# joyfang1106/MRLA

Measured on AMD Instinct MI355X. Metric: images/sec fwd+bwd resnet50_mrlal b=256, higher is better.
Workload: dtype bf16

## Files before the change

### include/mrla_hip.h

```cpp
#ifndef MRLA_HIP_H_
#define MRLA_HIP_H_

#include <stddef.h>
#include <stdint.h>

#ifdef __cplusplus
extern "C" {
#endif

#define MRLA_OK 0
#define MRLA_EINVAL (-1)
#define MRLA_EUNSUPPORTED (-2)
#define MRLA_EHIP (-3)

enum { MRLA_F32 = 0, MRLA_BF16 = 1, MRLA_F16 = 2 };
enum { MRLA_NCHW = 0, MRLA_NHWC = 1 };
enum { MRLA_ACT_NONE = 0, MRLA_ACT_GELU = 1 };
enum { MRLA_BN_NONE = 0, MRLA_BN_TRAIN = 1, MRLA_BN_EVAL = 2 };

#define MRLA_FWD_MOMENTS 8
#define MRLA_BWD_MOMENTS 3
#define MRLA_GEMM_MOMENTS 4

#define MRLA_ABI_VERSION 5
// ... 186 lines not shown
int mrla_conv1x1_rows(int m, int k, int n, int dtype);
int mrla_conv1x1_plan(int m, int k, int n, int dtype, int addend, int* out);
int mrla_conv1x1_fwd(const void* x, const void* w, void* y, float* mom_part, int m, int k, int n, int dtype, void* stream);

int mrla_conv1x1_add_supported(int m, int k, int n, int dtype);
int mrla_conv1x1_fwd_add(const void* x, const void* w, const void* addend, void* y, int m, int k, int n, int dtype,
                         void* stream);

int mrla_conv1x1_addend_supported(int m, int k, int n, int sh, int sw, int dtype);
int mrla_conv1x1_fwd_addend(const void* x, const void* w, const void* addend, void* y, int m, int k, int n, int b, int h,
                            int w_, int sh, int sw, int dtype, void* stream);

int mrla_conv1x1_fwd_affine_supported(int m, int k, int n, int dtype);
int mrla_conv1x1_fwd_affine(const void* x, const void* w, const float* sc, const float* sh, int relu, void* y, int m, int k,
                            int n, int dtype, void* stream);

int mrla_conv1x1_wgrad_rows(int m, int k, int n, int dtype);
int mrla_conv1x1_wgrad_plan(int m, int k, int n, int dtype, int* out);
int mrla_conv1x1_wgrad(const void* dy, const void* x, float* part, void* dw, int m, int k, int n, int dtype, int dw_dtype,
                       void* stream);

int mrla_conv1x1_wgrad_bn_supported(int m, int k, int n, int dtype);
int mrla_conv1x1_wgrad_bn(const void* g, const void* xb, const float* sc, const float* sh, const float* cb , int relu,
                          void* dy_out, const void* x, float* part, void* dw, int m, int k, int n, int dtype, int dw_dtype,
                          void* stream);

int mrla_conv1x1_wgrad_bn_dx_supported(int m, int k, int n, int dtype);
int mrla_conv1x1_wgrad_bn_dx(const void* g, const void* xb, const float* sc, const float* sh, const float* cb ,
                             int relu, const void* x, const void* wt , void* dx , float* part, void* dw,
                             int m, int k, int n, int dtype, int dw_dtype, void* stream);

int mrla_conv3x3_wgrad_rows(int b, int c, int n, int h, int w, int stride, int dtype);
int mrla_conv3x3_wgrad_plan(int b, int c, int n, int h, int w, int stride, int dtype, int* out);
int mrla_conv3x3_wgrad(const void* dy, const void* x, float* part, void* dw, int b, int c, int n, int h, int w,
                       int stride, int dtype, int dw_dtype, void* stream);

int mrla_conv3x3_fwd_rows(int b, int c, int n, int h, int w, int stride, int dtype);
int mrla_conv3x3_fwd_plan(int b, int c, int n, int h, int w, int stride, int dtype, int* out);
int mrla_conv3x3_fwd(const void* x, const void* wt, void* y, float* mom_part , int b, int c, int n, int h, int w,
                     int stride, int dtype, void* stream);

int mrla_conv3x3_dgrad_s2_plan(int b, int c, int n, int h, int w, int dtype, int* out);
int mrla_conv3x3_dgrad_s2(const void* dy, const void* wt, void* dx, int b, int c, int n, int h, int w, int dtype, void* stream);

int mrla_stem_conv_wgrad_rows(int b, int n, int h, int w, int dtype);
int mrla_stem_conv_wgrad_plan(int b, int n, int h, int w, int dtype, int* out);
int mrla_stem_conv_wgrad(const void* dy, const void* x, float* part, void* dw, int b, int n, int h, int w, int dtype,
                         int dw_dtype, void* stream);

int mrla_conv1x1_f32_rows(int m, int k, int n);
int mrla_conv1x1_f32_plan(int m, int k, int n, int* out);
int mrla_conv1x1_f32_fwd(const float* x, const float* w, int w_trans, float* y, float* mom_part , int m, int k, int n,
                         void* stream);
int mrla_conv1x1_f32_wgrad_rows(int m, int k, int n);
int mrla_conv1x1_f32_wgrad(const float* dy, const float* x, float* part, float* dw, int m, int k, int n, void* stream);

int mrla_weight_bank_refresh(const void* table, int entries, int max_tiles, void* stream);
int mrla_weight_bank_refresh_dt(const void* table, int entries, int max_tiles, int dtype, void* stream);

int mrla_reduce_rows(const float* in, float* out, int rows, int n, void* stream);
int mrla_reduce_rows2(const float* in1, float* out1, int rows1, int n1, const float* in2, float* out2, int rows2, int n2,
                      void* stream);



int mrla_light_tail_fwd(const void* x, const float* pre_sc, const float* pre_sh, const void* o_prev, const float* wq,
// ... 58 lines not shown
```

### mrla_amd/__init__.py

```python


def __getattr__(name):
    if name in ("graphed_step", "GraphedStep", "replay_matches_eager", "capture_step", "GraphReplayMismatch"):
        from . import graphs
        return getattr(graphs, name)
    if name == "fp32_gemms":
        from . import functional
        return functional.fp32_gemms
    if name == "conv3x3_wgrad":
        from . import functional
        return functional.conv3x3_wgrad
    if name == "conv3x3_fwd":
        from . import functional
        return functional.conv3x3_fwd
    if name == "conv3x3_dgrad":
        from . import functional
        return functional.conv3x3_dgrad
    if name == "stem_wgrad":
        from . import functional
        return functional.stem_wgrad
    if name == "reproducible_gradients":
        from . import functional
        return functional.reproducible_gradients
    raise AttributeError(f"module 'mrla_amd' has no attribute {name!r}")
```

### mrla_amd/_lib.py

```python
import ctypes
import os

_HERE = os.path.dirname(os.path.abspath(__file__))
LIB_PATH = os.environ.get("MRLA_HIP_LIB") or os.path.join(_HERE, "libmrla_hip.so")

ABI_VERSION = 5
OK, EINVAL, EUNSUPPORTED, EHIP = 0, -1, -2, -3
F32, BF16, F16 = 0, 1, 2
NCHW, NHWC = 0, 1
ACT_NONE, ACT_GELU = 0, 1
BN_NONE, BN_TRAIN, BN_EVAL = 0, 1, 2
FWD_MOMENTS, BWD_MOMENTS, TOKEN_PARTIALS, GEMM_MOMENTS = 8, 3, 15, 4

_ERR = {EINVAL: "invalid argument", EUNSUPPORTED: "unsupported shape/layout for the HIP kernels",
        EHIP: "HIP runtime error at kernel launch"}

_P, _I, _F = ctypes.c_void_p, ctypes.c_int, ctypes.c_float

SIGNATURES = {
    "mrla_abi_version": [],
    "mrla_light_wgrad_rows": [_I] * 6,
    "mrla_light_stats_fwd": [_P, _P, _P, _P, _I, _I, _I, _I, _I, _I, _I, _P],
    "mrla_light_gate_fwd": [_P, _P, _P, _I, _P, _I, _I, _I, _I, _P],
    "mrla_light_bn_fwd": [_P, _P, _P, _P, _P, _P, _P, _I, _F, _F, _P, _P, _P, _P, _I, _I, _I, _I, _P],
# ... 51 lines not shown
    "mrla_bn_relu_pool_fwd": [_P, _P, _P, _P, _I, _I, _I, _I, _I, _I, _P],
    "mrla_bn_relu_pool_dmoments": [_P, _P, _P, _P, _P, _P, _I, _I, _I, _I, _I, _I, _P],
    "mrla_bn_relu_pool_bwd": [_P, _P, _P, _P, _P, _P, _I, _I, _I, _I, _I, _I, _P],
    "mrla_bn_gate_supported": [_I] * 6,
    "mrla_bn_gate_pool": [_P] * 6 + [_I] * 5 + [_P],
    "mrla_eca_gate_fwd": [_P, _P, _I, _P, _I, _I, _P],
    "mrla_eca_gate_bwd": [_P, _P, _P, _P, _I, _P, _P, _P, _I, _I, _I, _P],
    "mrla_bn_gate_sums_bwd": [_P] * 9 + [_I] * 5 + [_P],
    "mrla_bn_gate_fwd": [_P, _P, _P, _P, _P] + [_I] * 6 + [_P],
    "mrla_bn_gate_bwd": [_P, _P, _P, _P, _P, _P] + [_I] * 6 + [_P],
    "mrla_conv1x1_rows": [_I] * 4,
    "mrla_conv1x1_plan": [_I, _I, _I, _I, _I, _P],
    "mrla_conv1x1_wgrad_plan": [_I, _I, _I, _I, _P],
    "mrla_conv1x1_fwd": [_P, _P, _P, _P, _I, _I, _I, _I, _P],
    "mrla_conv1x1_add_supported": [_I] * 4,
    "mrla_conv1x1_fwd_add": [_P, _P, _P, _P, _I, _I, _I, _I, _P],
    "mrla_conv1x1_addend_supported": [_I] * 6,
    "mrla_conv1x1_fwd_addend": [_P, _P, _P, _P] + [_I] * 9 + [_P],
    "mrla_conv1x1_fwd_affine_supported": [_I] * 4,
    "mrla_conv1x1_fwd_affine": [_P, _P, _P, _P, _I, _P, _I, _I, _I, _I, _P],
    "mrla_conv1x1_wgrad_rows": [_I] * 4,
    "mrla_conv1x1_wgrad": [_P, _P, _P, _P, _I, _I, _I, _I, _I, _P],
    "mrla_conv1x1_f32_rows": [_I] * 3,
    "mrla_conv1x1_f32_plan": [_I, _I, _I, _P],
    "mrla_conv1x1_f32_fwd": [_P, _P, _I, _P, _P, _I, _I, _I, _P],
    "mrla_conv1x1_f32_wgrad_rows": [_I] * 3,
    "mrla_conv1x1_f32_wgrad": [_P, _P, _P, _P, _I, _I, _I, _P],
    "mrla_conv1x1_wgrad_bn_supported": [_I] * 4,
    "mrla_conv1x1_wgrad_bn": [_P, _P, _P, _P, _P, _I, _P, _P, _P, _P, _I, _I, _I, _I, _I, _P],
    "mrla_conv1x1_wgrad_bn_dx_supported": [_I] * 4,
    "mrla_conv1x1_wgrad_bn_dx": [_P, _P, _P, _P, _P, _I, _P, _P, _P, _P, _P, _I, _I, _I, _I, _I, _P],
    "mrla_conv3x3_wgrad_rows": [_I] * 7,
    "mrla_conv3x3_wgrad_plan": [_I] * 7 + [_P],
    "mrla_conv3x3_wgrad": [_P, _P, _P, _P] + [_I] * 8 + [_P],
    "mrla_conv3x3_fwd_rows": [_I] * 7,
    "mrla_conv3x3_fwd_plan": [_I] * 7 + [_P],
    "mrla_conv3x3_fwd": [_P, _P, _P, _P] + [_I] * 7 + [_P],
    "mrla_conv3x3_dgrad_s2_plan": [_I] * 6 + [_P],
    "mrla_conv3x3_dgrad_s2": [_P, _P, _P] + [_I] * 6 + [_P],
    "mrla_stem_conv_wgrad_rows": [_I] * 5,
    "mrla_stem_conv_wgrad_plan": [_I] * 5 + [_P],
    "mrla_stem_conv_wgrad": [_P, _P, _P, _P] + [_I] * 6 + [_P],
    "mrla_weight_bank_refresh": [_P, _I, _I, _P],
    "mrla_weight_bank_refresh_dt": [_P, _I, _I, _I, _P],
    "mrla_reduce_rows": [_P, _P, _I, _I, _P],
    "mrla_reduce_rows2": [_P, _P, _I, _I, _P, _P, _I, _I, _P],
    "mrla_light_tail_fwd": [_P] * 6 + [_I] + [_P] * 6 + [_I, _F, _F] + [_P] * 6 + [_I] * 10 + [_P],
    "mrla_light_tail_bwd": [_P] * 5 + [_I] + [_P] * 7 + [_I] + [_P] * 5 + [_I] + [_P] * 8 + [_I] * 10 + [_P],
    "mrla_bn_fwd": [_P, _P, _I, _P, _P, _I, _P, _P, _P, _P, _I, _F, _F, _P, _I, _P] + [_I] * 6 + [_P],
    "mrla_bn_bwd": [_P] * 5 + [_I] * 4 + [_P, _P] + [_I] * 6 + [_P],
    "mrla_stem_fwd": [_P, _P, _P, _I, _P, _P, _P, _P, _I, _F, _F, _P, _P] + [_I] * 6 + [_P],
    "mrla_stem_bwd": [_P] * 5 + [_I, _I, _P, _P] + [_I] * 6 + [_P],
    "mrla_base_layer_fwd": [_P] * 6 + [_I] + [_P] * 5 + [_I, _F, _F] + [_P] * 9 + [_I] + [_P, _P] + [_I] * 9 + [_P],
    "mrla_base_layer_bwd": ([_P] * 5 + [_I] + [_P] * 6 + [_I] + [_P] * 6 + [_I] + [_P, _P] + [_I] + [_P] * 5 + [_I] + [_P] * 5
                            + [_I] * 12 + [_P]),
    "mrla_token_light_fwd": [_P] * 8 + [_I] + [_P, _P] + [_F] + [_P] * 4 + [_I] * 6 + [_P],
    "mrla_token_light_bwd": [_P] * 10 + [_I] + [_P] * 6 + [_I] + [_P] * 6 + [_I] * 6 + [_P],
}


class MrlaHipError(RuntimeError):
    pass


_lib = None

# ... 77 lines not shown
```

### mrla_amd/csrc/capi.hip

```cpp
#include <algorithm>
#include <atomic>
#include <mutex>

#include "mrla_device.h"
#include "mrla_kernels.h"

namespace mrla {

hipError_t lds_opt_in(const void* kernel, size_t bytes) {
  if (bytes <= 48 * 1024) return hipSuccess;
  constexpr unsigned kSlots = 1024;
  static std::atomic<uintptr_t> keys[kSlots];
  static std::atomic<int> granted[kSlots];
  static std::mutex raise_mutex;
  int dev = 0;
  if (hipGetDevice(&dev) != hipSuccess) return hipErrorInvalidDevice;
  const uintptr_t key = reinterpret_cast<uintptr_t>(kernel) ^ ((uintptr_t)(dev + 1) << 52);
  unsigned i = (unsigned)((key >> 4) * 0x9E3779B1u) % kSlots;
  int slot = -1;
  for (unsigned probe = 0; probe < kSlots; ++probe, i = (i + 1) % kSlots) {
    uintptr_t k = keys[i].load(std::memory_order_acquire);
    if (k == 0 && keys[i].compare_exchange_strong(k, key, std::memory_order_acq_rel)) k = key;
    if (k == key) { slot = (int)i; break; }
  }
// ... 712 lines not shown
  if ((dw_dtype == MRLA_F16 && dtype != MRLA_F16) || (dw_dtype == MRLA_BF16 && dtype == MRLA_F16)) return MRLA_EINVAL;
  if (dtype != MRLA_BF16 && dtype != MRLA_F16) return MRLA_EUNSUPPORTED;
  return launch_conv1x1_wgrad(dy, x, part, dw, dw_dtype == MRLA_F32, m, k, n, dtype, (hipStream_t)stream);
}

static int conv3x3_args(int b, int c, int n, int h, int w, int stride, int dtype) {
  if (b <= 0 || c <= 0 || n <= 0 || h <= 0 || w <= 0 || stride <= 0 || bad_dtype(dtype)) return MRLA_EINVAL;
  if (dtype != MRLA_BF16 && dtype != MRLA_F16) return MRLA_EUNSUPPORTED;
  return MRLA_OK;
}

static int stem_conv_wgrad_args(int b, int n, int h, int w, int dtype) { return conv3x3_args(b, 3, n, h, w, 2, dtype); }

static int wgrad_launch_args(const void* dy, const void* x, const void* part, const void* dw, int dtype, int dw_dtype, int rc) {
  if (!dy || !x || !part || !dw) return MRLA_EINVAL;
  if (((uintptr_t)dy | (uintptr_t)x | (uintptr_t)part | (uintptr_t)dw) & 15) return MRLA_EINVAL;
  if (dw_dtype != MRLA_BF16 && dw_dtype != MRLA_F16 && dw_dtype != MRLA_F32) return MRLA_EINVAL;
  if (rc == MRLA_EINVAL) return rc;
  if (dw_dtype != MRLA_F32 && dw_dtype != dtype) return MRLA_EINVAL;
  return rc;
}

int mrla_conv3x3_wgrad_rows(int b, int c, int n, int h, int w, int stride, int dtype) {
  const int rc = conv3x3_args(b, c, n, h, w, stride, dtype);
  return rc != MRLA_OK ? rc : conv3x3_wgrad_rows(b, c, n, h, w, stride);
}

int mrla_conv3x3_wgrad_plan(int b, int c, int n, int h, int w, int stride, int dtype, int* out) {
  if (!out) return MRLA_EINVAL;
  const int rc = conv3x3_args(b, c, n, h, w, stride, dtype);
  return rc != MRLA_OK ? rc : conv3x3_wgrad_plan(b, c, n, h, w, stride, out);
}

int mrla_conv3x3_wgrad(const void* dy, const void* x, float* part, void* dw, int b, int c, int n, int h, int w, int stride,
                       int dtype, int dw_dtype, void* stream) {
  const int rc = wgrad_launch_args(dy, x, part, dw, dtype, dw_dtype, conv3x3_args(b, c, n, h, w, stride, dtype));
  if (rc != MRLA_OK) return rc;
  return launch_conv3x3_wgrad(dy, x, part, dw, dw_dtype == MRLA_F32, b, c, n, h, w, stride, dtype, (hipStream_t)stream);
}

int mrla_conv3x3_fwd_rows(int b, int c, int n, int h, int w, int stride, int dtype) {
  const int rc = conv3x3_args(b, c, n, h, w, stride, dtype);
  return rc != MRLA_OK ? rc : conv3x3_fwd_rows(b, c, n, h, w, stride);
}

int mrla_conv3x3_fwd_plan(int b, int c, int n, int h, int w, int stride, int dtype, int* out) {
  if (!out) return MRLA_EINVAL;
  const int rc = conv3x3_args(b, c, n, h, w, stride, dtype);
  return rc != MRLA_OK ? rc : conv3x3_fwd_plan(b, c, n, h, w, stride, out);
}

int mrla_conv3x3_fwd(const void* x, const void* wt, void* y, float* mom_part, int b, int c, int n, int h, int w, int stride,
                     int dtype, void* stream) {
  if (!x || !wt || !y) return MRLA_EINVAL;
  if (((uintptr_t)x | (uintptr_t)wt | (uintptr_t)y | (uintptr_t)mom_part) & 15) return MRLA_EINVAL;
  const int rc = conv3x3_args(b, c, n, h, w, stride, dtype);
  if (rc != MRLA_OK) return rc;
  return launch_conv3x3_fwd(x, wt, y, mom_part, b, c, n, h, w, stride, dtype, (hipStream_t)stream);
}

int mrla_conv3x3_dgrad_s2_plan(int b, int c, int n, int h, int w, int dtype, int* out) {
  if (!out) return MRLA_EINVAL;
  const int rc = conv3x3_args(b, c, n, h, w, 2, dtype);
  return rc != MRLA_OK ? rc : conv3x3_dgrad_s2_plan(b, c, n, h, w, out);
}

// ... 180 lines not shown
```

### mrla_amd/csrc/conv3x3_wgrad.hip

```cpp
#include <algorithm>
#include <type_traits>

#include "conv_spatial.h"

namespace mrla {
namespace {

typedef c1_f32x16 c3_f32x16;

constexpr int kC3Tile = 64;
constexpr int kC3Waves = 4;
constexpr int kC3Stages = 1;
constexpr int kC3Target = 2 * 256;
constexpr int kC3MaxKP1 = 128;
constexpr int kC3MaxKP2 = 96;
constexpr int kC3MaxPY = 60;
static_assert(kTileRowB == kC3Tile * 2, "a tile row is one pixel, 64 channels");

struct C3Plan : Raster3x3 {
  int rows_per_split = 0, splits = 0, tiles = 0;
};

struct C3Args {
  int b, h, w, ho, wo, c, n;
  int py, ws, nseg, rmax, kp_cap;
  int rows_per_split, splits, tiles_c;
  float inv_py, inv_px;
};

__device__ __forceinline__ int c3_off(int row, int chunk) { return tile_off<1, 2>(row, chunk); }

template <typename T>
__device__ __forceinline__ typename Elem16<T>::x8 c3_frag(const unsigned char* tile, int r, int r2, int chunk, int sub) {
  return tr16_frag<T>(tile + c3_off(r, chunk) + sub, tile + c3_off(r2, chunk) + sub);
}

template <typename T, int S>
__device__ __forceinline__ void conv3x3_wgrad_body(const T* __restrict__ dY, const T* __restrict__ X, float* __restrict__ part,
                                                   const C3Args& a) {
#if defined(__HIP_DEVICE_COMPILE__)
  extern __shared__ __align__(16) unsigned char smem_raw[];
  unsigned char* const ty_tile = smem_raw;
  unsigned char* const tx_tile = smem_raw + a.kp_cap * kTileRowB;
  const int tid = threadIdx.x, lane = tid & (kWave - 1), wave = tid / kWave;
  const int tiles = (a.n / kC3Tile) * a.tiles_c;
  const int split = blockIdx.x / tiles, tile = blockIdx.x - split * tiles;
  const int tn = tile / a.tiles_c, tc = tile - tn * a.tiles_c;
  const int n0 = tn * kC3Tile, c0 = tc * kC3Tile;
  const int rows = a.b * a.ho;
  const int r_begin = split * a.rows_per_split, r_end = min(rows, r_begin + a.rows_per_split);
  const int PY = a.py, PX = S * a.py;

  const int wn = wave >> 1, wc = wave & 1;
  const int g = lane >> 4, q = (lane >> 2) & 3, pp = lane & 3;
  const int krel = 8 * (g >> 1) + q;
  const int colA = wn * 32 + 16 * (g & 1) + 4 * pp, colB = wc * 32 + 16 * (g & 1) + 4 * pp;
  const int chA = colA >> 3, subA = ((colA >> 2) & 1) * 8, chB = colB >> 3, subB = ((colB >> 2) & 1) * 8;

  c3_f32x16 acc[9];
#pragma unroll
  for (int t = 0; t < 9; ++t)
#pragma unroll
    for (int e = 0; e < 16; ++e) acc[t][e] = 0.f;

  const int prow = tid >> 3, pch = tid & 7;
  const u32x4 zero4 = {0u, 0u, 0u, 0u};

  for (int r = r_begin; r < r_end;) {
    const RowStep st = row_step(r, r_end, a.ho, a.rmax);
    const int img = st.img, yo0 = st.yo0, R = st.R;
    for (int seg = 0; seg < a.nseg; ++seg) {
      const int xo0 = seg * a.ws, ws = min(a.ws, a.wo - xo0);
      const int KP = (R * PY + 15) & ~15;
      const int XT = S * KP + S * (S - 1) * PY * (R - 1) + 2 * PX + 3;
      const int ty_need = S * (R - 1) + 3, cx_need = S * (ws - 1) + 3;
      const int yi0 = yo0 * S - 1, xi0 = xo0 * S - 1;
      __syncthreads();
      for (int p0 = 0; p0 < KP; p0 += 128) {
        u32x4 v[4];
#pragma unroll
        for (int u = 0; u < 4; ++u) {
          const int p = p0 + 32 * u + prow;
          const int ry = (int)(((float)p + 0.5f) * a.inv_py), j = p - ry * PY;
          v[u] = zero4;
          if (p < KP && ry < R && j < ws)
            v[u] = *reinterpret_cast<const u32x4*>(dY + ((size_t)((img * a.ho + yo0 + ry) * a.wo + xo0 + j) * a.n + n0 + pch * 8));
        }
#pragma unroll
        for (int u = 0; u < 4; ++u) {
          const int p = p0 + 32 * u + prow;
          if (p < KP) *reinterpret_cast<u32x4*>(ty_tile + c3_off(p, pch)) = v[u];
        }
      }
      for (int t0 = 0; t0 < XT; t0 += 128) {
        u32x4 v[4];
#pragma unroll
        for (int u = 0; u < 4; ++u) {
          const int t = t0 + 32 * u + prow;
          const int ty = (int)(((float)t + 0.5f) * a.inv_px), cx = t - ty * PX;
          const int yi = yi0 + ty, xi = xi0 + cx;
          v[u] = zero4;
          if (t < XT && ty < ty_need && cx < cx_need && yi >= 0 && yi < a.h && xi >= 0 && xi < a.w)
            v[u] = *reinterpret_cast<const u32x4*>(X + ((size_t)((img * a.h + yi) * a.w + xi) * a.c + c0 + pch * 8));
        }
#pragma unroll
        for (int u = 0; u < 4; ++u) {
          const int t = t0 + 32 * u + prow;
          if (t < XT) *reinterpret_cast<u32x4*>(tx_tile + c3_off(t, pch)) = v[u];
        }
      }
      __syncthreads();
      for (int k0 = 0; k0 < KP; k0 += 16) {
        const int k = k0 + krel;
        const typename Elem16<T>::x8 fa = c3_frag<T>(ty_tile, k, k + 4, chA, subA);
        int xr = S * k, xr2 = S * (k + 4);
        if (S > 1) {
          xr += S * (S - 1) * PY * min((int)(((float)k + 0.5f) * a.inv_py), R - 1);
          xr2 += S * (S - 1) * PY * min((int)(((float)k + 4.5f) * a.inv_py), R - 1);
        }
#pragma unroll
        for (int kh = 0; kh < 3; ++kh)
#pragma unroll
          for (int kw = 0; kw < 3; ++kw) {
            const typename Elem16<T>::x8 fb = c3_frag<T>(tx_tile, xr + kh * PX + kw, xr2 + kh * PX + kw, chB, subB);
            Elem16<T>::mfma(acc[kh * 3 + kw], fa, fb);
          }
      }
    }
    r += R;
  }

  float* po = part + (((size_t)split * a.n + n0 + wn * 32) * 9) * a.c + c0 + wc * 32 + (lane & 31);
  const int hh = lane >> 5;
#pragma unroll
  for (int t = 0; t < 9; ++t)
#pragma unroll
    for (int e = 0; e < 16; ++e) po[((size_t)(8 * (e >> 2) + 4 * hh + (e & 3)) * 9 + t) * a.c] = acc[t][e];
#endif
}

template <typename T, int S>
__global__ __launch_bounds__(kC3Waves* kWave, 2) void conv3x3_wgrad_kernel(const T* __restrict__ dY, const T* __restrict__ X,
                                                                           float* __restrict__ part, C3Args a) {
  conv3x3_wgrad_body<T, S>(dY, X, part, a);
}

C3Plan c3_plan(int b, int c, int n, int h, int w, int s) {
  C3Plan p;
  static_cast<Raster3x3&>(p) = raster3x3(b, c, n, h, w, s, kC3MaxKP1, kC3MaxKP2, kC3MaxPY, 16);
  if (!p.ok) return p;
  p.tiles = (n / kC3Tile) * (c / kC3Tile);
  const RowSplit sp = split_rows((long long)b * p.ho, p.tiles, kC3Target);
  p.rows_per_split = sp.per;
  p.splits = sp.count;
  return p;
}

template <typename T, int S>
int c3_launch(const C3Plan& p, const C3Args& a, const void* dy, const void* x, float* part, hipStream_t st) {
  const size_t lds = (size_t)(p.kp_cap + p.xt_cap) * kTileRowB;
  if (lds > 80 * 1024) return MRLA_EUNSUPPORTED;
  if (lds_opt_in(reinterpret_cast<const void*>(conv3x3_wgrad_kernel<T, S>), lds) != hipSuccess) return MRLA_EHIP;
  hipLaunchKernelGGL((conv3x3_wgrad_kernel<T, S>), dim3(p.tiles * p.splits), dim3(kC3Waves * kWave), lds, st, (const T*)dy,
                     (const T*)x, part, a);
  return MRLA_OK;
}

}

int conv3x3_wgrad_rows(int b, int c, int n, int h, int w, int s) {
  const C3Plan p = c3_plan(b, c, n, h, w, s);
  return p.ok ? p.splits : MRLA_EUNSUPPORTED;
}

int conv3x3_wgrad_plan(int b, int c, int n, int h, int w, int s, int* out) {
  const C3Plan p = c3_plan(b, c, n, h, w, s);
  if (!p.ok) return MRLA_EUNSUPPORTED;
  out[0] = kC3Tile; out[1] = kC3Tile; out[2] = p.rows_per_split; out[3] = kC3Stages; out[4] = p.splits; out[5] = p.tiles;
  return MRLA_OK;
}

int launch_conv3x3_wgrad(const void* dy, const void* x, float* part, void* dw, int dw_f32, int b, int c, int n, int h, int w,
                         int s, int dtype, hipStream_t st) {
  const C3Plan p = c3_plan(b, c, n, h, w, s);
  if (!p.ok || (dtype != MRLA_BF16 && dtype != MRLA_F16)) return MRLA_EUNSUPPORTED;
  C3Args a;
  a.b = b; a.h = h; a.w = w; a.ho = p.ho; a.wo = p.wo; a.c = c; a.n = n;
  a.py = p.py; a.ws = p.ws; a.nseg = p.nseg; a.rmax = p.rmax; a.kp_cap = p.kp_cap;
  a.rows_per_split = p.rows_per_split; a.splits = p.splits; a.tiles_c = c / kC3Tile;
  a.inv_py = 1.0f / (float)p.py; a.inv_px = 1.0f / (float)(s * p.py);
  int rc;
  if (dtype == MRLA_F16)
    rc = s == 1 ? c3_launch<f16_t, 1>(p, a, dy, x, part, st) : c3_launch<f16_t, 2>(p, a, dy, x, part, st);
  else
    rc = s == 1 ? c3_launch<bf16_t, 1>(p, a, dy, x, part, st) : c3_launch<bf16_t, 2>(p, a, dy, x, part, st);
  if (rc != MRLA_OK) return rc;
  return launch_split_sum(part, dw, dw_f32, dtype, p.splits, n * 9 * c, st);
}

}
```

### mrla_amd/csrc/mrla_kernels.h

```cpp
#pragma once
#include <hip/hip_runtime.h>
#include <stddef.h>
#include <stdint.h>

#include "../../include/mrla_hip.h"

namespace mrla {

constexpr int kMaxTasksPerWave = 4;

struct SlabGeo {
  int B, C, H, W, HW;
  int CP;
  int slabs;
  int WS;
  int PW;
  int NG;
  int NB;
  int RB;
  int BG;
  int astride;
};

inline size_t dtype_size(int dtype) { return dtype == MRLA_F32 ? 4 : 2; }
// ... 146 lines not shown
int launch_bn_relu_pool_bwd(const void* dp, const void* x, const float* sc, const float* sh, const float* cb, void* dx,
                            int B, int C, int H, int W, int dtype, hipStream_t st);
int conv1x1_wide_rows(int M, int K, int N);
int conv1x1_wide_plan(int M, int K, int N, int add, int* out);
int launch_conv1x1_wide(const void* x, const void* w, const void* addend, void* y, float* part, int M, int K, int N,
                        int dtype, hipStream_t st);
int launch_conv1x1_wide_sparse(const void* x, const void* w, const void* addend, void* y, int M, int K, int N, int b, int h,
                               int wd, int sh, int sw, int dtype, hipStream_t st);
int launch_conv1x1_wide_affine(const void* x, const void* w, const float* sc, const float* sh, int relu, void* y, int M, int K,
                               int N, int dtype, hipStream_t st);
int conv1x1_kstream_supported(int M, int K, int N);
int conv1x1_kstream_stages(int M, int K, int N);
int conv1x1_kstream_rows(int M, int K, int N);
int launch_conv1x1_kstream(const void* x, const void* w, void* y, float* part, int M, int K, int N, int dtype, hipStream_t st);
int launch_conv1x1_kstream_addend(const void* x, const void* w, const void* addend, void* y, int M, int K, int N, int b, int h,
                                  int wd, int sh, int sw, int dtype, hipStream_t st);
int launch_conv1x1_kstream_affine(const void* x, const void* w, const float* sc, const float* sh, int relu, void* y, int M,
                                  int K, int N, int dtype, hipStream_t st);
int conv1x1_wgrad_rows(int M, int K, int N);
int conv1x1_wgrad_plan(int M, int K, int N, int* out);
int launch_conv1x1_wgrad(const void* dy, const void* x, float* part, void* dw, int dw_f32, int M, int K, int N, int dtype,
                         hipStream_t st);
int conv1x1_wgrad_bn_supported(int M, int K, int N);
int launch_conv1x1_wgrad_bn(const void* g, const void* xb, const float* sc, const float* sh, const float* cb, int relu,
                            void* dy_out, const void* x, float* part, void* dw, int dw_f32, int M, int K, int N, int dtype,
                            hipStream_t st);
int conv1x1_wgrad_bn_dx_supported(int M, int K, int N);
int launch_conv1x1_wgrad_bn_dx(const void* g, const void* xb, const float* sc, const float* sh, const float* cb, int relu,
                               const void* x, const void* wt, void* dx, float* part, void* dw, int dw_f32, int M, int K, int N,
                               int dtype, hipStream_t st);
int launch_conv1x1_wgrad_reduce_f32(const float* part, float* dw, int splits, int NK, hipStream_t st);
int conv3x3_wgrad_rows(int b, int c, int n, int h, int w, int s);
int conv3x3_wgrad_plan(int b, int c, int n, int h, int w, int s, int* out);
int launch_conv3x3_wgrad(const void* dy, const void* x, float* part, void* dw, int dw_f32, int b, int c, int n, int h, int w,
                         int s, int dtype, hipStream_t st);
int conv3x3_fwd_rows(int b, int c, int n, int h, int w, int s);
int conv3x3_fwd_plan(int b, int c, int n, int h, int w, int s, int* out);
int launch_conv3x3_fwd(const void* x, const void* wt, void* y, float* mom, int b, int c, int n, int h, int w, int s, int dtype,
                       hipStream_t st);
int conv3x3_dgrad_s2_plan(int b, int c, int n, int h, int w, int* out);
int launch_conv3x3_dgrad_s2(const void* dy, const void* wt, void* dx, int b, int c, int n, int h, int w, int dtype,
                            hipStream_t st);
int stem_conv_wgrad_rows(int b, int n, int h, int w);
int stem_conv_wgrad_plan(int b, int n, int h, int w, int* out);
int launch_stem_conv_wgrad(const void* dy, const void* x, float* part, void* dw, int dw_f32, int b, int n, int h, int w,
                           int dtype, hipStream_t st);
int conv1x1_f32_rows(int M, int K, int N);
int conv1x1_f32_plan(int M, int K, int N, int* out);
int launch_conv1x1_f32_fwd(const float* x, const float* w, int w_trans, float* y, float* part, int M, int K, int N,
                           hipStream_t st);
int conv1x1_f32_wgrad_rows(int M, int K, int N);
int launch_conv1x1_f32_wgrad(const float* dy, const float* x, float* part, float* dw, int M, int K, int N, hipStream_t st);
int launch_weight_bank_refresh(const long long* table, int entries, int max_tiles, int dtype, hipStream_t st);
int launch_light_stats_fwd_wide(const void* x, const void* o, const float* wv, float* mom, void* xout, const float* psc,
                                const float* psh, void* vout, int B, int C, int H, int W, int dtype, int act,
                                hipStream_t st, bool fused_no_x = false, int mom_ranges = 1);
int launch_light_apply_fwd_wide(const void* x, const void* o, const float* wv, const float* gate, const float* sc,
                                const float* sh, const float* lam, const float* dp, void* out, int B, int C, int H,
                                int W, int d, int res, int dtype, int act, hipStream_t st);
int launch_light_apply_fwd_pre_wide(const void* pre, const void* o, const float* psc, const float* psh, const float* wv,
                                    const float* gate, const float* sc, const float* sh, const float* lam,
                                    const float* dp, void* out, int B, int C, int H, int W, int d, int res, int dtype,
                                    hipStream_t st);
int launch_light_apply_bwd_wide(const void* dout, const void* x, const void* o, const float* wv, const float* gate,
                                const float* cb, const float* lam, const float* dp, const float* dyx, void* dx,
                                void* dprev, float* dwv_part, const void* pre, const float* pre_center, float* pre_tmom,
// ... 50 lines not shown
```

### mrla_amd/functional.py

```python
import contextlib
import ctypes
import threading
import weakref
from math import log

import torch

from . import _lib as L

_DT = {torch.float32: L.F32, torch.bfloat16: L.BF16, torch.float16: L.F16}


def k_size_for(c):
    t = int(abs((log(c, 2) + 1) / 2.0))
    return t if t % 2 else t + 1


class KernelTimer:

    def __init__(self, names=None):
        self.names = None if names is None else set(names)
        self.records = []

    def summary(self):
# ... 15 lines not shown
LEAN = False


SHORTCUT_ADDEND = True


WGRAD_BN = True


CONV1X1_F32 = False


def _switch(flag, name):
    @contextlib.contextmanager
    def manager(enabled=True):
        g = globals()
        prev, g[flag] = g[flag], bool(enabled)
        try:
            yield
        finally:
            g[flag] = prev
    manager.__name__ = manager.__qualname__ = name
    manager.__doc__ = f"{flag} = `enabled` inside the block; the previous value comes back on exit, also when the block raises."
    return manager


fp32_gemms = _switch("CONV1X1_F32", "fp32_gemms")


CONV3X3_WGRAD = False


conv3x3_wgrad = _switch("CONV3X3_WGRAD", "conv3x3_wgrad")


CONV3X3_FWD = False


conv3x3_fwd = _switch("CONV3X3_FWD", "conv3x3_fwd")


CONV3X3_DGRAD = False


conv3x3_dgrad = _switch("CONV3X3_DGRAD", "conv3x3_dgrad")


STEM_WGRAD = False


stem_wgrad = _switch("STEM_WGRAD", "stem_wgrad")


@contextlib.contextmanager
def reproducible_gradients(enabled=True):
    with conv3x3_wgrad(enabled), stem_wgrad(enabled):
        yield


WGRAD_BN_DX = True


CHANNEL_GATE = True


EVAL_FOLD = True
# ... 1692 lines not shown
        return None
    n, (kh, kw, c) = dy.shape[1], taps
    part = torch.empty((rows, n, kh * kw * c), dtype=torch.float32, device=x.device)
    gw = torch.empty((n, c, kh, kw), dtype=ctx.wdtype, device=x.device, memory_format=_CL)
    _call(entry, (dy.numel() + x.numel()) * x.element_size(), _ptr(dy), _ptr(x), _ptr(part), _ptr(gw), *shape, dt,
          _DT[ctx.wdtype], _stream())
    return gw


def _stock_conv_backward(ctx, dy, x, w16, stride, padding, gx, gw):
    need_x, need_w = ctx.needs_input_grad[0] and gx is None, ctx.needs_input_grad[1] and gw is None
    if need_x or need_w:
        gx2, gw2, _ = torch.ops.aten.convolution_backward(dy, x, w16, None, stride, padding, (1, 1), False, (0, 0), 1,
                                                          [need_x, need_w, False])
        gx = gx2 if need_x else gx
        gw = gw2.to(ctx.wdtype) if need_w else gw
    return gx, gw


def _weight_strides(ctx, gw):
    if gw is not None and gw.stride() != ctx.wstride:
        gw = torch.empty_strided(ctx.wshape, ctx.wstride, dtype=gw.dtype, device=gw.device).copy_(gw)
    return gw


def conv3x3_applies(conv, x):
    dt = _spatial_conv_applies(conv, x, (3, 3), ((1, 1), (2, 2)), (1, 1), True)
    if dt is None:
        return False
    b, c, h, w = x.shape
    return L.load().mrla_conv3x3_wgrad_rows(b, c, conv.out_channels, h, w, conv.stride[0], _DT[dt]) > 0


def _own_dgrad_s2(dy, x, w16):
    b, c, h, wd = x.shape
    gx = torch.empty_like(x)
    _call("mrla_conv3x3_dgrad_s2", (dy.numel() + gx.numel()) * x.element_size(), _ptr(dy), _ptr(w16), _ptr(gx),
          b, c, w16.shape[0], h, wd, _DT[x.dtype], _stream())
    return gx


class _Conv3x3Fn(torch.autograd.Function):

    @staticmethod
    @_on_device
    def forward(ctx, x, w, stride, own_wgrad, own_dgrad):
        ctx.stride, ctx.own_wgrad, ctx.own_dgrad = (stride, stride), own_wgrad, own_dgrad
        ctx.wshape, ctx.wstride, ctx.wdtype = w.shape, w.stride(), w.dtype
        w16 = w if w.dtype == x.dtype else w.to(x.dtype)
        if own_dgrad:
            w16 = w16.contiguous(memory_format=_CL)
            if w16.data_ptr() % 16:
                w16 = w16.clone(memory_format=_CL)
        ctx.save_for_backward(x, w16)
        return torch.ops.aten.convolution(x, w16, None, ctx.stride, (1, 1), (1, 1), False, (0, 0), 1)

    @staticmethod
    @_on_device
    def backward(ctx, dy):
        x, w16 = ctx.saved_tensors
        dy = dy.contiguous(memory_format=_CL)
        b, c, h, wd = x.shape
        own = dy.dtype == x.dtype and dy.data_ptr() % 16 == 0
        gx = gw = None
        if ctx.needs_input_grad[1] and own and ctx.own_wgrad:
            gw = _own_wgrad(ctx, "mrla_conv3x3_wgrad", "mrla_conv3x3_wgrad_rows", dy, x,
# ... 44 lines not shown
              _ptr(part) if moments else None, b, c, n, h, wd, stride, dt, _stream())
        ctx.save_for_backward(x, w16)
        ctx.mark_non_differentiable(part)
        return y, part

    @staticmethod
    @_on_device
    def backward(ctx, dy, _dpart=None):
        if dy is None:
            return None, None, None, None, None, None
        x, w16 = ctx.saved_tensors
        need_x, need_w = ctx.needs_input_grad[0], ctx.needs_input_grad[1]
        dy = dy.contiguous(memory_format=_CL)
        b, c, h, wd = x.shape
        n, dt = w16.shape[0], _DT[x.dtype]
        own = dy.dtype == x.dtype and dy.data_ptr() % 16 == 0
        gx = gw = None
        if need_w and own and ctx.own_wgrad:
            gw = _own_wgrad(ctx, "mrla_conv3x3_wgrad", "mrla_conv3x3_wgrad_rows", dy, x, (b, c, n, h, wd, ctx.stride[0]), (3, 3, c))
        if need_x and own and ctx.stride[0] == 1:
            wflip = w16.flip(2, 3).transpose(0, 1).contiguous(memory_format=_CL)
            gx = torch.empty_like(x)
            _call("mrla_conv3x3_fwd", (dy.numel() + gx.numel()) * x.element_size(), _ptr(dy), _ptr(wflip), _ptr(gx), None,
                  b, n, c, h, wd, 1, dt, _stream())
        if need_x and own and ctx.own_dgrad:
            gx = _own_dgrad_s2(dy, x, w16)
        gx, gw = _stock_conv_backward(ctx, dy, x, w16, ctx.stride, (1, 1), gx, gw)
        return gx, _weight_strides(ctx, gw), None, None, None, None


def _conv3x3_own(x, conv, moments):
    dt = _conv_compute_dtype(x)
    return _Conv3x3FwdFn.apply(x if x.dtype == dt else x.to(dt), conv.weight, conv.stride[0], moments,
                               CONV3X3_WGRAD and conv3x3_applies(conv, x), CONV3X3_DGRAD and conv3x3_dgrad_applies(conv, x))


def conv3x3(x, conv):
    if CONV3X3_FWD and conv3x3_fwd_applies(conv, x):
        return _conv3x3_own(x, conv, False)[0]
    own_wgrad = CONV3X3_WGRAD and conv3x3_applies(conv, x)
    own_dgrad = CONV3X3_DGRAD and conv3x3_dgrad_applies(conv, x)
    if not (own_wgrad or own_dgrad):
        return conv(x)
    dt = _conv_compute_dtype(x)
    return _Conv3x3Fn.apply(x if x.dtype == dt else x.to(dt), conv.weight, conv.stride[0], own_wgrad, own_dgrad)


def conv3x3_bn_act(x, conv, bn, relu, defer=False):
    if CONV3X3_FWD and conv3x3_fwd_applies(conv, x):
        moments = type(bn) is torch.nn.BatchNorm2d and bn.affine and bn.track_running_stats and bn.training
        y, part = _conv3x3_own(x, conv, moments)
        return bn_act(y, bn, relu, defer, pre_moments=part if moments else None)
    return bn_act(conv3x3(x, conv), bn, relu, defer)


def stem_conv_applies(conv, x):
    dt = _spatial_conv_applies(conv, x, (7, 7), ((2, 2),), (3, 3), True)
    if dt is None or conv.in_channels != 3:
        return False
    b, _, h, w = x.shape
    return L.load().mrla_stem_conv_wgrad_rows(b, conv.out_channels, h, w, _DT[dt]) > 0


class _StemConvFn(torch.autograd.Function):

    @staticmethod
    @_on_device
    def forward(ctx, x, w):
        ctx.wshape, ctx.wstride, ctx.wdtype = w.shape, w.stride(), w.dtype
        w16 = w if w.dtype == x.dtype else w.to(x.dtype)
        ctx.save_for_backward(x, w16)
        return torch.ops.aten.convolution(x, w16, None, (2, 2), (3, 3), (1, 1), False, (0, 0), 1)

# ... 104 lines not shown
```

Before: 9181.

## Prefetch next conv3x3 wgrad step and auto-enable kernel for stride-1 shapes

Restructures the conv3x3 weight-gradient kernel so the dY and X tiles for the next row/segment step are loaded into registers while the current step's MFMAs run. For stride 1 the X raster comes entirely from that register prefetch. The stride-1 inner loop is rewritten to load the B fragment for the next tap ahead of its MFMA. A heuristic (steps ≥ 4, pixels ≥ 384, stride 1) exposed through a new C API now turns the custom wgrad on by default for stride-1 convs instead of the stock PyTorch backward. The trade-off is more register pressure and a dispatch decision cached per shape.

```diff
diff --git a/include/mrla_hip.h b/include/mrla_hip.h
--- a/include/mrla_hip.h
+++ b/include/mrla_hip.h
@@ -242,6 +242,7 @@
 
 int mrla_conv3x3_wgrad_rows(int b, int c, int n, int h, int w, int stride, int dtype);
 int mrla_conv3x3_wgrad_plan(int b, int c, int n, int h, int w, int stride, int dtype, int* out);
+int mrla_conv3x3_wgrad_preferred(int b, int c, int n, int h, int w, int stride, int dtype);
 int mrla_conv3x3_wgrad(const void* dy, const void* x, float* part, void* dw, int b, int c, int n, int h, int w,
                        int stride, int dtype, int dw_dtype, void* stream);
 
diff --git a/mrla_amd/__init__.py b/mrla_amd/__init__.py
--- a/mrla_amd/__init__.py
+++ b/mrla_amd/__init__.py
@@ -10,6 +10,9 @@
     if name == "conv3x3_wgrad":
         from . import functional
         return functional.conv3x3_wgrad
+    if name == "conv3x3_wgrad_auto":
+        from . import functional
+        return functional.conv3x3_wgrad_auto
     if name == "conv3x3_fwd":
         from . import functional
         return functional.conv3x3_fwd
diff --git a/mrla_amd/_lib.py b/mrla_amd/_lib.py
--- a/mrla_amd/_lib.py
+++ b/mrla_amd/_lib.py
@@ -107,6 +107,7 @@
     "mrla_conv1x1_wgrad_bn_dx": [_P, _P, _P, _P, _P, _I, _P, _P, _P, _P, _P, _I, _I, _I, _I, _I, _P],
     "mrla_conv3x3_wgrad_rows": [_I] * 7,
     "mrla_conv3x3_wgrad_plan": [_I] * 7 + [_P],
+    "mrla_conv3x3_wgrad_preferred": [_I] * 7,
     "mrla_conv3x3_wgrad": [_P, _P, _P, _P] + [_I] * 8 + [_P],
     "mrla_conv3x3_fwd_rows": [_I] * 7,
     "mrla_conv3x3_fwd_plan": [_I] * 7 + [_P],
diff --git a/mrla_amd/csrc/capi.hip b/mrla_amd/csrc/capi.hip
--- a/mrla_amd/csrc/capi.hip
+++ b/mrla_amd/csrc/capi.hip
@@ -768,6 +768,11 @@
   return rc != MRLA_OK ? rc : conv3x3_wgrad_plan(b, c, n, h, w, stride, out);
 }
 
+int mrla_conv3x3_wgrad_preferred(int b, int c, int n, int h, int w, int stride, int dtype) {
+  const int rc = conv3x3_args(b, c, n, h, w, stride, dtype);
+  return rc != MRLA_OK ? rc : conv3x3_wgrad_preferred(b, c, n, h, w, stride);
+}
+
 int mrla_conv3x3_wgrad(const void* dy, const void* x, float* part, void* dw, int b, int c, int n, int h, int w, int stride,
                        int dtype, int dw_dtype, void* stream) {
   const int rc = wgrad_launch_args(dy, x, part, dw, dtype, dw_dtype, conv3x3_args(b, c, n, h, w, stride, dtype));
diff --git a/mrla_amd/csrc/conv3x3_wgrad.hip b/mrla_amd/csrc/conv3x3_wgrad.hip
--- a/mrla_amd/csrc/conv3x3_wgrad.hip
+++ b/mrla_amd/csrc/conv3x3_wgrad.hip
@@ -50,6 +50,10 @@
   const int rows = a.b * a.ho;
   const int r_begin = split * a.rows_per_split, r_end = min(rows, r_begin + a.rows_per_split);
   const int PY = a.py, PX = S * a.py;
+  constexpr int kYPieces = S == 1 ? 4 : 3, kPreX = S == 1 ? 2 : 1;
+  constexpr bool kXAllPre = S == 1;
+  static_assert(kC3MaxKP1 <= 128 && kC3MaxKP2 <= 96, "the dY raster of a step is one pass of the loader");
+  static_assert(kC3MaxKP1 + 2 * kC3MaxPY + 3 <= 256, "the X raster of a stride-1 step is two passes of the loader");
 
   const int wn = wave >> 1, wc = wave & 1;
   const int g = lane >> 4, q = (lane >> 2) & 3, pp = lane & 3;
@@ -65,59 +69,115 @@
 
   const int prow = tid >> 3, pch = tid & 7;
   const u32x4 zero4 = {0u, 0u, 0u, 0u};
-
-  for (int r = r_begin; r < r_end;) {
+  const unsigned char* const dYb = reinterpret_cast<const unsigned char*>(dY);
+  const unsigned char* const Xb = reinterpret_cast<const unsigned char*>(X);
+
+  struct Seg {
+    int r, seg, img, yo0, R, xo0, ws;
+  };
+  auto seg_at = [&](int r, int seg) {
     const RowStep st = row_step(r, r_end, a.ho, a.rmax);
-    const int img = st.img, yo0 = st.yo0, R = st.R;
-    for (int seg = 0; seg < a.nseg; ++seg) {
-      const int xo0 = seg * a.ws, ws = min(a.ws, a.wo - xo0);
-      const int KP = (R * PY + 15) & ~15;
-      const int XT = S * KP + S * (S - 1) * PY * (R - 1) + 2 * PX + 3;
-      const int ty_need = S * (R - 1) + 3, cx_need = S * (ws - 1) + 3;
-      const int yi0 = yo0 * S - 1, xi0 = xo0 * S - 1;
-      __syncthreads();
-      for (int p0 = 0; p0 < KP; p0 += 128) {
+    Seg g;
+    g.r = r; g.seg = seg; g.img = st.img; g.yo0 = st.yo0; g.R = st.R;
+    g.xo0 = seg * a.ws; g.ws = min(a.ws, a.wo - g.xo0);
+    return g;
+  };
+  auto load_y = [&](const Seg& g, u32x4 (&v)[kYPieces]) {
+    const int KP = (g.R * PY + 15) & ~15;
+#pragma unroll
+    for (int u = 0; u < kYPieces; ++u) {
+      int p = 32 * u + prow;
+      v[u] = zero4;
+      if (p < KP) {
+        asm volatile("" : "+v"(p));
+        const int ry = (int)(((float)p + 0.5f) * a.inv_py), j = p - ry * PY;
+        if (ry < g.R && j < g.ws)
+          v[u] = *reinterpret_cast<const u32x4*>(dYb + 2u * (unsigned)(((g.img * a.ho + g.yo0 + ry) * a.wo + g.xo0 + j) * a.n + n0 + pch * 8));
+      }
+    }
+  };
+  auto load_x = [&](const Seg& g, int pass, u32x4 (&v)[4]) {
+    const int KP = (g.R * PY + 15) & ~15;
+    const int XT = S * KP + S * (S - 1) * PY * (g.R - 1) + 2 * PX + 3;
+    const int ty_need = S * (g.R - 1) + 3, cx_need = S * (g.ws - 1) + 3;
+    const int yi0 = g.yo0 * S - 1, xi0 = g.xo0 * S - 1;
+#pragma unroll
+    for (int u = 0; u < 4; ++u) {
+      int t = 128 * pass + 32 * u + prow;
+      v[u] = zero4;
+      if (t < XT) {
+        asm volatile("" : "+v"(t));
+        const int ty = (int)(((float)t + 0.5f) * a.inv_px), cx = t - ty * PX;
+        const int yi = yi0 + ty, xi = xi0 + cx;
+        if (ty < ty_need && cx < cx_need && yi >= 0 && yi < a.h && xi >= 0 && xi < a.w)
+          v[u] = *reinterpret_cast<const u32x4*>(Xb + 2u * (unsigned)(((g.img * a.h + yi) * a.w + xi) * a.c + c0 + pch * 8));
+      }
+    }
+  };
+  auto store_x = [&](int XT, int pass, const u32x4 (&v)[4]) {
+#pragma unroll
+    for (int u = 0; u < 4; ++u) {
+      const int t = 128 * pass + 32 * u + prow;
+      if (t < XT) *reinterpret_cast<u32x4*>(tx_tile + c3_off(t, pch)) = v[u];
+    }
+  };
+
+  u32x4 vy[kYPieces], vx[kPreX > 0 ? kPreX : 1][4];
+  Seg cur = seg_at(r_begin, 0);
+  bool more = r_begin < r_end;
+  if (more) {
+    load_y(cur, vy);
+#pragma unroll
+    for (int i = 0; i < kPreX; ++i) load_x(cur, i, vx[i]);
+  }
+  while (more) {
+    const int R = cur.R;
+    const int KP = (R * PY + 15) & ~15;
+    const int XT = S * KP + S * (S - 1) * PY * (R - 1) + 2 * PX + 3;
+    __syncthreads();
+#pragma unroll
+    for (int u = 0; u < kYPieces; ++u) {
+      const int p = 32 * u + prow;
+      if (p < KP) *reinterpret_cast<u32x4*>(ty_tile + c3_off(p, pch)) = vy[u];
+    }
+#pragma unroll
+    for (int i = 0; i < kPreX; ++i) store_x(XT, i, vx[i]);
+    if (!kXAllPre)
+      for (int pass = kPreX; pass * 128 < XT; ++pass) {
         u32x4 v[4];
-#pragma unroll
-        for (int u = 0; u < 4; ++u) {
-          const int p = p0 + 32 * u + prow;
-          const int ry = (int)(((float)p + 0.5f) * a.inv_py), j = p - ry * PY;
-          v[u] = zero4;
-          if (p < KP && ry < R && j < ws)
-            v[u] = *reinterpret_cast<const u32x4*>(dY + ((size_t)((img * a.ho + yo0 + ry) * a.wo + xo0 + j) * a.n + n0 + pch * 8));
+        load_x(cur, pass, v);
+        store_x(XT, pass, v);
+      }
+    __syncthreads();
+    Seg nxt = cur;
+    more = cur.seg + 1 < a.nseg || cur.r + R < r_end;
+    if (more) {
+      nxt = cur.seg + 1 < a.nseg ? seg_at(cur.r, cur.seg + 1) : seg_at(cur.r + R, 0);
+      load_y(nxt, vy);
+#pragma unroll
+      for (int i = 0; i < kPreX; ++i) load_x(nxt, i, vx[i]);
+    }
+    for (int k0 = 0; k0 < KP; k0 += 16) {
+      const int k = k0 + krel;
+      const typename Elem16<T>::x8 fa = c3_frag<T>(ty_tile, k, k + 4, chA, subA);
+      int xr = S * k, xr2 = S * (k + 4);
+      if (S > 1) {
+        xr += S * (S - 1) * PY * min((int)(((float)k + 0.5f) * a.inv_py), R - 1);
+        xr2 += S * (S - 1) * PY * min((int)(((float)k + 4.5f) * a.inv_py), R - 1);
+      }
+      if constexpr (S == 1) {
+        typename Elem16<T>::x8 fb = c3_frag<T>(tx_tile, xr, xr2, chB, subB);
+#pragma unroll
+        for (int t = 0; t < 9; ++t) {
+          typename Elem16<T>::x8 fbn = fb;
+          if (t < 8) {
+            const int off = ((t + 1) / 3) * PX + (t + 1) % 3;
+            fbn = c3_frag<T>(tx_tile, xr + off, xr2 + off, chB, subB);
+          }
+          Elem16<T>::mfma(acc[t], fa, fb);
+          fb = fbn;
         }
-#pragma unroll
-        for (int u = 0; u < 4; ++u) {
-          const int p = p0 + 32 * u + prow;
-          if (p < KP) *reinterpret_cast<u32x4*>(ty_tile + c3_off(p, pch)) = v[u];
-        }
-      }
-      for (int t0 = 0; t0 < XT; t0 += 128) {
-        u32x4 v[4];
-#pragma unroll
-        for (int u = 0; u < 4; ++u) {
-          const int t = t0 + 32 * u + prow;
-          const int ty = (int)(((float)t + 0.5f) * a.inv_px), cx = t - ty * PX;
-          const int yi = yi0 + ty, xi = xi0 + cx;
-          v[u] = zero4;
-          if (t < XT && ty < ty_need && cx < cx_need && yi >= 0 && yi < a.h && xi >= 0 && xi < a.w)
-            v[u] = *reinterpret_cast<const u32x4*>(X + ((size_t)((img * a.h + yi) * a.w + xi) * a.c + c0 + pch * 8));
-        }
-#pragma unroll
-        for (int u = 0; u < 4; ++u) {
-          const int t = t0 + 32 * u + prow;
-          if (t < XT) *reinterpret_cast<u32x4*>(tx_tile + c3_off(t, pch)) = v[u];
-        }
-      }
-      __syncthreads();
-      for (int k0 = 0; k0 < KP; k0 += 16) {
-        const int k = k0 + krel;
-        const typename Elem16<T>::x8 fa = c3_frag<T>(ty_tile, k, k + 4, chA, subA);
-        int xr = S * k, xr2 = S * (k + 4);
-        if (S > 1) {
-          xr += S * (S - 1) * PY * min((int)(((float)k + 0.5f) * a.inv_py), R - 1);
-          xr2 += S * (S - 1) * PY * min((int)(((float)k + 4.5f) * a.inv_py), R - 1);
-        }
+      } else {
 #pragma unroll
         for (int kh = 0; kh < 3; ++kh)
 #pragma unroll
@@ -127,7 +187,7 @@
           }
       }
     }
-    r += R;
+    cur = nxt;
   }
 
   float* po = part + (((size_t)split * a.n + n0 + wn * 32) * 9) * a.c + c0 + wc * 32 + (lane & 31);
@@ -178,6 +238,15 @@
   if (!p.ok) return MRLA_EUNSUPPORTED;
   out[0] = kC3Tile; out[1] = kC3Tile; out[2] = p.rows_per_split; out[3] = kC3Stages; out[4] = p.splits; out[5] = p.tiles;
   return MRLA_OK;
+}
+
+constexpr int kC3PreferSteps = 4, kC3PreferPixels = 384;
+int conv3x3_wgrad_preferred(int b, int c, int n, int h, int w, int s) {
+  const C3Plan p = c3_plan(b, c, n, h, w, s);
+  if (!p.ok) return MRLA_EUNSUPPORTED;
+  const long long steps = (long long)((p.rows_per_split + p.rmax - 1) / p.rmax) * p.nseg;
+  const long long pixels = (long long)p.rows_per_split * p.wo;
+  return s == 1 && steps >= kC3PreferSteps && pixels >= kC3PreferPixels;
 }
 
 int launch_conv3x3_wgrad(const void* dy, const void* x, float* part, void* dw, int dw_f32, int b, int c, int n, int h, int w,
diff --git a/mrla_amd/csrc/mrla_kernels.h b/mrla_amd/csrc/mrla_kernels.h
--- a/mrla_amd/csrc/mrla_kernels.h
+++ b/mrla_amd/csrc/mrla_kernels.h
@@ -202,6 +202,7 @@
 int launch_conv1x1_wgrad_reduce_f32(const float* part, float* dw, int splits, int NK, hipStream_t st);
 int conv3x3_wgrad_rows(int b, int c, int n, int h, int w, int s);
 int conv3x3_wgrad_plan(int b, int c, int n, int h, int w, int s, int* out);
+int conv3x3_wgrad_preferred(int b, int c, int n, int h, int w, int s);
 int launch_conv3x3_wgrad(const void* dy, const void* x, float* part, void* dw, int dw_f32, int b, int c, int n, int h, int w,
                          int s, int dtype, hipStream_t st);
 int conv3x3_fwd_rows(int b, int c, int n, int h, int w, int s);
diff --git a/mrla_amd/functional.py b/mrla_amd/functional.py
--- a/mrla_amd/functional.py
+++ b/mrla_amd/functional.py
@@ -71,6 +71,12 @@
 
 
 conv3x3_wgrad = _switch("CONV3X3_WGRAD", "conv3x3_wgrad")
+
+
+CONV3X3_WGRAD_AUTO = True
+
+
+conv3x3_wgrad_auto = _switch("CONV3X3_WGRAD_AUTO", "conv3x3_wgrad_auto")
 
 
 CONV3X3_FWD = False
@@ -1829,6 +1835,22 @@
     return L.load().mrla_conv3x3_wgrad_rows(b, c, conv.out_channels, h, w, conv.stride[0], _DT[dt]) > 0
 
 
+_WGRAD_PREFERRED = {}
+
+
+def _conv3x3_own_wgrad(conv, x):
+    if not ((CONV3X3_WGRAD or CONV3X3_WGRAD_AUTO) and conv3x3_applies(conv, x)):
+        return False
+    if CONV3X3_WGRAD:
+        return True
+    b, c, h, w = x.shape
+    key = (b, c, conv.out_channels, h, w, conv.stride[0], _DT[_conv_compute_dtype(x)])
+    hit = _WGRAD_PREFERRED.get(key)
+    if hit is None:
+        hit = _WGRAD_PREFERRED[key] = L.load().mrla_conv3x3_wgrad_preferred(*key) == 1
+    return hit
+
+
 def _own_dgrad_s2(dy, x, w16):
     b, c, h, wd = x.shape
     gx = torch.empty_like(x)
@@ -1939,13 +1961,13 @@
 def _conv3x3_own(x, conv, moments):
     dt = _conv_compute_dtype(x)
     return _Conv3x3FwdFn.apply(x if x.dtype == dt else x.to(dt), conv.weight, conv.stride[0], moments,
-                               CONV3X3_WGRAD and conv3x3_applies(conv, x), CONV3X3_DGRAD and conv3x3_dgrad_applies(conv, x))
+                               _conv3x3_own_wgrad(conv, x), CONV3X3_DGRAD and conv3x3_dgrad_applies(conv, x))
 
 
 def conv3x3(x, conv):
     if CONV3X3_FWD and conv3x3_fwd_applies(conv, x):
         return _conv3x3_own(x, conv, False)[0]
-    own_wgrad = CONV3X3_WGRAD and conv3x3_applies(conv, x)
+    own_wgrad = _conv3x3_own_wgrad(conv, x)
     own_dgrad = CONV3X3_DGRAD and conv3x3_dgrad_applies(conv, x)
     if not (own_wgrad or own_dgrad):
         return conv(x)
```

New measurement: 9337 (median of 6 runs). 1.02x the previous value.
